# filixi/TCP-stack

Hardware: AMD Instinct MI355X
Metric: GiB/s device-resident TCP checksum over batched segments; % HBM roofline (higher is better)
Workload: dtype u16; 1 GPU; C2: 1M x 1460-B payload (1492-B images), fixed stride, device-resident; images_per_gpu=1048576, image_bytes=1492, bytes_per_gpu=1564475392, parallelism=shard1 (independent per-GPU batches, no collective)

## Files before the change

tcp-stack_amd/csrc/tcpck_device.h:

```cpp
#pragma once

#include <hip/hip_runtime.h>
#include <stdint.h>

#include "tcpck_internal.h"

namespace tcpck {
namespace dev {

using u32x4 = __attribute__((ext_vector_type(4))) unsigned int;

constexpr int kBlock = 256;
constexpr int kWavesPerBlock = kBlock / 64;

template <typename Kernel>
inline uint32_t resident_blocks_per_cu(Kernel kernel) {
  int nb = 0;
  if (hipOccupancyMaxActiveBlocksPerMultiprocessor(&nb, kernel, kBlock, 0) != hipSuccess || nb < 1) nb = 1;
  return static_cast<uint32_t>(nb);
}

inline uint32_t oversub_for(uint32_t requested, uint64_t bytes, uint64_t resident_waves, uint32_t max_m,
                            uint32_t min_run = 4u << 10) {
  if (requested) return requested;
// ... 78 lines not shown
  const uint32_t s = acc + w;
  return s + (s < w ? 1u : 0u);
}

template <int MODE>
__device__ __forceinline__ uint32_t accumulate(uint32_t acc, uint32_t w) {
  if constexpr (MODE == kRef) {
    return ref_add(acc, w);
  } else {
    return rfc_add(acc, w);
  }
}

template <int MODE>
__device__ __forceinline__ uint32_t fold_lane(uint32_t acc) {
  if constexpr (MODE == kRef) {
    return acc & 0xFFFFu;
  } else {
    acc = (acc & 0xFFFFu) + (acc >> 16);
    return (acc & 0xFFFFu) + (acc >> 16);
  }
}

template <int MODE>
__device__ __forceinline__ uint16_t finish(uint32_t sum) {
  if constexpr (MODE == kRef) {
    return static_cast<uint16_t>(~sum);
  } else {
    sum = (sum & 0xFFFFu) + (sum >> 16);
    sum = (sum & 0xFFFFu) + (sum >> 16);
    return static_cast<uint16_t>(~sum);
  }
}

template <int G>
__device__ __forceinline__ uint32_t group_sum(uint32_t x) {
#pragma unroll
  for (int m = G / 2; m >= 1; m >>= 1) x += __shfl_xor(x, m, 64);
  return x;
}

__device__ __forceinline__ uint32_t wave_inclusive_scan(uint32_t x) {
  x += __builtin_amdgcn_update_dpp(0, x, 0x111, 0xF, 0xF, false);
  x += __builtin_amdgcn_update_dpp(0, x, 0x112, 0xF, 0xF, false);
  x += __builtin_amdgcn_update_dpp(0, x, 0x114, 0xF, 0xF, false);
  x += __builtin_amdgcn_update_dpp(0, x, 0x118, 0xF, 0xF, false);
  x += __builtin_amdgcn_update_dpp(0, x, 0x142, 0xA, 0xF, false);
  x += __builtin_amdgcn_update_dpp(0, x, 0x143, 0xC, 0xF, false);
  return x;
}

__device__ __forceinline__ uint32_t read_lane(uint32_t x, uint32_t lane) {
  return static_cast<uint32_t>(__builtin_amdgcn_readlane(static_cast<int>(x), static_cast<int>(lane)));
}

__device__ __forceinline__ uint64_t read_lane64(uint64_t x, uint32_t lane) {
  const uint32_t lo = read_lane(static_cast<uint32_t>(x), lane);
  const uint32_t hi = read_lane(static_cast<uint32_t>(x >> 32), lane);
  return (static_cast<uint64_t>(hi) << 32) | lo;
}

template <bool EXACT = false>
__device__ __forceinline__ uint32_t words_before(uint32_t r, uint32_t x, uint32_t y, uint32_t z, uint32_t w) {
  const uint32_t nw = r >> 1;
  uint32_t h = 0;
  auto both = [](uint32_t d) -> uint32_t { return EXACT ? (d & 0xFFFFu) + (d >> 16) : d + (d >> 16); };
  if (nw >= 2) h += both(x);
  if (nw >= 4) h += both(y);
  if (nw >= 6) h += both(z);
  if (nw & 1) {
    const uint32_t d = nw == 1 ? x : (nw == 3 ? y : (nw == 5 ? z : w));
    h += d & 0xFFFFu;
  }
  return h;
}

template <int U, int MODE>
__device__ __forceinline__ uint32_t wave_image_sum(const uint8_t *arena, uint64_t start, uint32_t len,
                                                   bool exclude_field) {
  const uint32_t lane = threadIdx.x & 63;
  const uint64_t a0 = align16_rel(arena, start);
  const uint8_t *p0 = arena + a0;
  const int32_t lead = static_cast<int32_t>(start - a0);
  const int64_t span64 = lead + static_cast<int64_t>(len);
  const uint32_t nch = static_cast<uint32_t>((span64 + 15) >> 4);
  const int64_t field = exclude_field ? lead + 28 : -64;
  uint32_t acc = 0;
  for (uint32_t i0 = lane; i0 < nch; i0 += 64 * U) {
    u32x4 v[U];
#pragma unroll
    for (int u = 0; u < U; ++u) {
      const uint32_t i = i0 + u * 64;
      v[u] = load16_nt(p0 + 16 * static_cast<uint64_t>(i < nch ? i : nch - 1));
    }
#pragma unroll
    for (int u = 0; u < U; ++u) {
      const int64_t rel = 16 * static_cast<int64_t>(i0 + u * 64);
      const int32_t lo = static_cast<int32_t>(min(max(lead - rel, int64_t{0}), int64_t{16}));
      const int32_t hi = static_cast<int32_t>(min(max(span64 - rel, int64_t{0}), int64_t{16}));
      uint32_t wm = word_mask(lo, hi);
      const int64_t fb = field - rel;
      if (fb >= 0 && fb < 16) wm &= ~(1u << (fb >> 1));
      u32x4 w = v[u];
      if (wm != 0xFFu) w = apply_mask(w, wm);
      acc = accumulate<MODE>(acc, w.x);
      acc = accumulate<MODE>(acc, w.y);
// ... 27 lines not shown
                                         uint64_t t1, uint64_t &r0, uint64_t &r1) {
  const uint32_t lane = threadIdx.x & 63;
  uint64_t lo[2] = {0, 0}, hi[2] = {count, count};
  const uint64_t t[2] = {t0, t1};
  while (hi[0] - lo[0] > 64 || hi[1] - lo[1] > 64) {
    uint64_t step[2], idx[2], v[2];
#pragma unroll
    for (int i = 0; i < 2; ++i) {
      step[i] = hi[i] - lo[i] > 64 ? (hi[i] - lo[i] + 63) / 64 : 1;
      idx[i] = lo[i] + lane * step[i];
      v[i] = idx[i] < hi[i] ? offsets[idx[i]] : 0;
    }
#pragma unroll
    for (int i = 0; i < 2; ++i) {
      if (hi[i] - lo[i] <= 64) continue;
      const bool below = idx[i] < hi[i] && v[i] - base < t[i];
      const uint32_t c = __popcll(__ballot(below));
      const uint64_t nlo = c ? lo[i] + (c - 1) * step[i] + 1 : lo[i];
      hi[i] = min(hi[i], lo[i] + c * step[i]);
      lo[i] = nlo;
    }
  }
  uint64_t v[2];
#pragma unroll
  for (int i = 0; i < 2; ++i) {
    const uint64_t idx = lo[i] + lane;
    v[i] = idx < hi[i] ? offsets[idx] : 0;
  }
  const bool b0 = lo[0] + lane < hi[0] && v[0] - base < t0;
  const bool b1 = lo[1] + lane < hi[1] && v[1] - base < t1;
  r0 = lo[0] + __popcll(__ballot(b0));
  r1 = lo[1] + __popcll(__ballot(b1));
}

__device__ __forceinline__ void count_split(uint64_t wid, uint64_t q, uint64_t r, uint64_t &kb, uint64_t &ke) {
  kb = wid * q + (wid < r ? wid : r);
  ke = kb + q + (wid < r ? 1u : 0u);
}

__device__ __forceinline__ uint32_t xcd_block(uint32_t b, uint32_t nb) {
  const uint32_t q = nb >> 3, r = nb & 7u, x = b & 7u;
  return (x < r ? x * (q + 1) : r * (q + 1) + (x - r) * q) + (b >> 3);
}

__device__ __forceinline__ uint32_t xcd_chunk_block(uint32_t b, uint32_t nb, uint32_t lc) {
  const uint32_t full = (nb >> (3 + lc)) << (3 + lc);
  if (b >= full) return b;
  const uint32_t i = b >> 3;
  return ((((i >> lc) << 3) + (b & 7u)) << lc) + (i & ((1u << lc) - 1u));
}

constexpr uint32_t kOrderDefault = 0xFFu;
constexpr uint32_t kOrderXcd = 0xFEu;
__device__ __forceinline__ uint32_t ordered_block(uint32_t b, uint32_t nb, uint32_t lc) {
  if (lc == kOrderDefault) return b;
  if (lc == kOrderXcd) return xcd_block(b, nb);
  return xcd_chunk_block(b, nb, lc);
}


}
}
```

tcp-stack_amd/csrc/tcpck_internal.h:

```cpp
#pragma once

#include <hip/hip_runtime.h>
#include <stdint.h>

namespace tcpck {

enum Op : int { kChecksum = 0, kFill = 1, kVerify = 2 };
enum Mode : int { kRef = 0, kRfc1071 = 1 };

enum SegShape : int {
  kShapeSmall = 0,
  kShapeMss = 1,
  kShapeJumbo = 2,
  kShapeWave2 = 3,
  kShapeG32 = 4,
  kShapeG4 = 5,
  kShapeW4 = 6,
  kShapeW8 = 7,
  kShapeW16 = 8,
  kShapeW16U4 = 9,
  kShapeW2 = 10,
  kNumShapes = 11
};

struct SegArgs {
  uint8_t *arena;
  const uint64_t *offsets;
  const uint32_t *lengths;
  uint64_t stride;
  uint64_t base;
  uint64_t count;
  void *out;
  uint32_t len;
  uint32_t oversub;
  uint32_t order;
  uint32_t rot;
};

SegShape shape_for_len(uint64_t typical_len);
hipError_t launch_seg(int op, int mode, bool fixed, SegShape shape, const SegArgs &a,
                      uint32_t num_cus, hipStream_t stream);

struct RunArgs {
  uint8_t *arena;
  const uint64_t *offsets;
  const uint32_t *lengths;
  uint64_t stride;
  uint32_t len;
  uint64_t base;
  uint64_t count;
  void *out;
  uint32_t oversub;
  uint64_t total_bytes;
  uint32_t blocks_per_cu;
  int mode;
  uint8_t *hdr;
  uint64_t *dbg;
};

struct FixedStreamArgs {
  uint8_t *arena;
  uint64_t stride;
  uint64_t count;
  void *out;
  uint64_t *dbg;
  uint32_t blocks_per_cu;
  uint32_t oversub;
  uint64_t per_wave;
  uint64_t rem;
  uint32_t order;
  int mode;
  uint32_t defer_field;
  uint8_t *side;
  uint32_t side_nt;
};

struct GroupStreamArgs {
  uint8_t *arena;
  uint32_t len;
  uint64_t count;
  void *out;
  uint32_t oversub;
  uint32_t order;
  uint64_t per_wave;
  uint64_t rem;
};
bool gstream_applies(const uint8_t *arena, uint64_t stride, uint32_t len);
constexpr int kGstreamDefaultLoads = 0x80;
constexpr int kGstreamWriteBack = 0x401;
hipError_t launch_gstream(int op, int variant, const GroupStreamArgs &a, uint32_t num_cus, hipStream_t stream);

hipError_t launch_rstream(int op, int variant, const FixedStreamArgs &a, uint32_t num_cus, hipStream_t stream);
hipError_t launch_vvstream(int op, int variant, bool fixed, const RunArgs &a, uint32_t num_cus, hipStream_t stream);
hipError_t launch_rvstream(int op, int variant, const RunArgs &a, uint32_t num_cus, hipStream_t stream);
bool sstream_fixed_applies(uint64_t stride, uint32_t len);
hipError_t launch_sstream(int op, int variant, bool fixed, const RunArgs &a, uint32_t num_cus, hipStream_t stream);
struct SegmentArgs {
  const uint8_t *payload;
  uint8_t *images;
  uint64_t payload_bytes;
  uint64_t count;
  uint16_t *out;
  uint64_t per_wave, rem;
  uint32_t seg;
  uint32_t stride;
  uint32_t nchunk, magic, shift;
  uint32_t hdr[8];
  uint32_t seq0;
  uint32_t order;
};
hipError_t launch_segment(int mode, int variant, SegmentArgs a, uint32_t oversub, uint32_t num_cus,
                          hipStream_t stream);
struct AckArgs {
  uint8_t *arena;
  const uint64_t *offsets;
  uint64_t stride;
  uint64_t count;
  const uint32_t *acks;
  uint32_t ack;
  uint16_t *out;
};
hipError_t launch_set_ack(int mode, const AckArgs &a, uint32_t num_cus, hipStream_t stream);

// ... 35 lines not shown
```

tcp-stack_amd/csrc/tcpck_rstream.hip:

```cpp
#include "tcpck_device.h"

namespace tcpck {

namespace {

using dev::kBlock;
using dev::kWavesPerBlock;
using dev::u32x4;

template <int U, int OP, bool STAMP, int PRIO = 0, int FLAV = 0, int MODE = kRef>
__global__ void __launch_bounds__(kBlock) rstream_kernel(FixedStreamArgs a) {
  constexpr bool SECT = OP == kFill && (FLAV & 32) != 0;
  __shared__ u32x4 s_sec[kWavesPerBlock][SECT ? 32 * 4 : 1];
  const uint32_t lane = threadIdx.x & 63;
  const uint32_t wv = static_cast<uint32_t>(__builtin_amdgcn_readfirstlane(static_cast<int>(threadIdx.x >> 6)));
  const uint32_t bid = dev::ordered_block(blockIdx.x, gridDim.x, a.order);
  const uint64_t wid = static_cast<uint64_t>(bid) * kWavesPerBlock +
                       static_cast<uint32_t>(__builtin_amdgcn_readfirstlane(static_cast<int>(threadIdx.x >> 6)));
  uint64_t t_start = 0;
  if (STAMP) t_start = __builtin_amdgcn_s_memrealtime();
  if (PRIO) {
    uint32_t hw;
    asm volatile("s_getreg_b32 %0, hwreg(HW_REG_HW_ID)" : "=s"(hw));
    const uint32_t slot = hw & 0xFu;
    if (PRIO == 1) {
      if (slot >= 6) {
        __builtin_amdgcn_s_setprio(3);
      } else if (slot >= 4) {
        __builtin_amdgcn_s_setprio(2);
      } else if (slot >= 2) {
        __builtin_amdgcn_s_setprio(1);
      }
    } else if (slot >= 4) {
      __builtin_amdgcn_s_setprio(1);
    }
  }
  uint64_t kb, ke;
  dev::count_split(wid, a.per_wave, a.rem, kb, ke);
  if (kb >= ke) return;
  const uint32_t S = static_cast<uint32_t>(a.stride);
  const uint64_t s0 = kb * S;
  const uint64_t A0 = dev::align128_rel(a.arena, s0);
  const uint32_t lead = static_cast<uint32_t>(s0 - A0);
  const uint32_t span = lead + static_cast<uint32_t>(ke - kb) * S;
  const uint32_t nsteps = (span + 1023) >> 10;
  const uint32_t last_chunk = (span - 1) >> 4;
  const uint8_t *base = a.arena + A0;

  const auto rsrc = dev::make_rsrc(base, (last_chunk + 1) << 4);
  uint32_t nl = lead + 28;
  auto load_step = [&](uint32_t st) -> u32x4 {
    if constexpr ((FLAV & 128) != 0 && OP == kFill) {
      const uint32_t sb = st << 10;
      uint64_t m = 0;
      while (nl < sb + 1024 && nl < span) {
        m |= uint64_t{0xF} << (((nl & ~63u) - sb) >> 4);
        nl += S;
      }
      if ((m >> lane) & 1u) {
        typedef unsigned v4u __attribute__((ext_vector_type(4)));
        const v4u v = __builtin_amdgcn_raw_buffer_load_b128(rsrc, static_cast<int>(lane << 4), static_cast<int>(sb), 0);
        return u32x4{v.x, v.y, v.z, v.w};
      }
      return dev::load16_buf_nt(rsrc, lane << 4, sb);
    } else if constexpr (FLAV & 2) {
      if constexpr (FLAV & 8) {
        typedef unsigned v4u __attribute__((ext_vector_type(4)));
        const v4u v = __builtin_amdgcn_raw_buffer_load_b128(rsrc, static_cast<int>(lane << 4), static_cast<int>(st << 10), 0);
        return u32x4{v.x, v.y, v.z, v.w};
      } else {
        return dev::load16_buf_nt(rsrc, lane << 4, st << 10);
      }
    } else {
      const uint32_t ci = min((st << 6) + lane, last_chunk);
      return dev::load16_nt(base + 16 * static_cast<uint64_t>(ci));
    }
  };

  const uint32_t nimg = static_cast<uint32_t>(ke - kb);
  uint32_t nb = lead + S;
  uint32_t jn = 1;
  uint32_t nf = lead + 28;
  uint32_t jf = 0;
  uint32_t fstage = 0;
  uint32_t ns = lead + 28;
  uint32_t js = 0;
  const bool end_flush = SECT && (FLAV & 64) != 0 && nimg <= 32;
  uint32_t carry = 0;
  uint32_t p_last = 0;
  uint32_t stage = 0;
  uint32_t out_rel = 0;

  auto flush = [&](uint32_t n) {
    if (lane < n) {
      const uint64_t k = kb + out_rel + lane;
      const uint16_t c = static_cast<uint16_t>(stage);
      if constexpr (OP == kVerify) {
        static_cast<uint8_t *>(a.out)[k] = (c == 0) ? 1 : 0;
      } else {
        if (a.out) static_cast<uint16_t *>(a.out)[k] = c;
// ... 108 lines not shown
        }
      }
      const uint32_t tot = (FLAV & 1) ? dev::ref_chunk_sum_dot(w) : dev::ref_chunk_sum(w);
      const uint32_t incl = dev::wave_inclusive_scan(tot);
      while (nb < sb + 1024 && jn < nimg) {
        const uint32_t rel = nb - sb;
        const uint32_t lb = rel >> 4;
        const uint32_t r = rel & 15u;
        uint32_t P = carry + dev::read_lane(incl, lb) - dev::read_lane(tot, lb);
        if (r)
          P += dev::words_before<MODE == kRfc1071>(r, dev::read_lane(w.x, lb), dev::read_lane(w.y, lb), dev::read_lane(w.z, lb),
                            dev::read_lane(w.w, lb));
        emit(jn - 1, P - p_last);
        p_last = P;
        nb += S;
        ++jn;
      }
      carry += dev::read_lane(incl, 63);
      ring[u] = load_step(st + U);
    }
  }
  emit(nimg - 1, carry - p_last);
  if constexpr (SECT) {
    if (end_flush) {
      for (uint32_t j0 = 0; j0 < nimg; j0 += 16) flush_sect(j0, min(nimg - j0, 16u));
    } else if (nimg & 15u) {
      flush_sect(nimg & ~15u, nimg & 15u);
    }
  }
  const uint32_t pending = nimg - out_rel;
  if (pending) flush(pending);
  if (STAMP && lane == 0 && a.dbg) {
    uint32_t hw_id, xcc_id;
    asm volatile("s_getreg_b32 %0, hwreg(HW_REG_HW_ID)" : "=s"(hw_id));
    asm volatile("s_getreg_b32 %0, hwreg(HW_REG_XCC_ID)" : "=s"(xcc_id));
    a.dbg[4 * wid] = t_start;
    a.dbg[4 * wid + 1] = __builtin_amdgcn_s_memrealtime();
    a.dbg[4 * wid + 2] = hw_id;
    a.dbg[4 * wid + 3] = xcc_id;
  }
}

template <int U, int OP, bool STAMP, int PRIO = 0, int FLAV = 0, int MODE = kRef>
hipError_t launch_one(const FixedStreamArgs &a, uint32_t num_cus, hipStream_t stream) {
  static const uint32_t per_cu = dev::resident_blocks_per_cu(rstream_kernel<U, OP, STAMP, PRIO, FLAV, MODE>);
  const uint32_t cap = (a.blocks_per_cu && a.blocks_per_cu < per_cu) ? a.blocks_per_cu : per_cu;
  const uint64_t resident = static_cast<uint64_t>(cap) * num_cus;
  uint64_t blocks = resident * dev::oversub_for(a.oversub, a.count * a.stride, resident * kWavesPerBlock, 1024);
  const uint64_t need = (a.count + kWavesPerBlock - 1) / kWavesPerBlock;
  if (!a.oversub && a.stride >= 3584 && a.count < 2 * blocks * kWavesPerBlock) blocks = need;
  if (blocks > need) blocks = need;
  if (blocks == 0) return hipSuccess;
  FixedStreamArgs b = a;
  b.per_wave = a.count / (blocks * kWavesPerBlock);
  b.rem = a.count % (blocks * kWavesPerBlock);
  hipLaunchKernelGGL((rstream_kernel<U, OP, STAMP, PRIO, FLAV, MODE>), dim3(static_cast<uint32_t>(blocks)), dim3(kBlock), 0,
                     stream, b);
  return hipGetLastError();
}

template <int U, bool STAMP, int PRIO = 0, int FLAV = 0, int MODE = kRef>
hipError_t dispatch(int op, const FixedStreamArgs &a, uint32_t num_cus, hipStream_t s) {
  switch (op) {
    case kChecksum: return launch_one<U, kChecksum, STAMP, PRIO, FLAV, MODE>(a, num_cus, s);
    case kFill: return launch_one<U, kFill, STAMP, PRIO, FLAV, MODE>(a, num_cus, s);
    case kVerify: return launch_one<U, kVerify, STAMP, PRIO, FLAV, MODE>(a, num_cus, s);
    default: return hipErrorInvalidValue;
  }
}

}

hipError_t launch_rstream(int op, int variant, const FixedStreamArgs &a, uint32_t num_cus, hipStream_t stream) {
  if (a.stride < 16 || a.count == 0) return hipErrorInvalidValue;
  const uint64_t max_run = ((a.count + 2047) / 2048 + 1) * a.stride + 128;
  if (max_run >= (uint64_t{1} << 31)) return hipErrorInvalidValue;
  if (a.mode != kRef) {
    if (variant != 20 || a.stride >= (1u << 17)) return hipErrorInvalidValue;
    FixedStreamArgs b = a;
    b.order = 4u;
    return dispatch<4, false, 0, 263, kRfc1071>(op, b, num_cus, stream);
  }
  if (variant == 20) {
    FixedStreamArgs b = a;
    b.order = 4u;
    return dispatch<4, false, 0, 263>(op, b, num_cus, stream);
  }
#ifdef TCPCK_PROBE
  switch (variant) {
    case 0: return dispatch<4, false>(op, a, num_cus, stream);
    case 1: return dispatch<2, false>(op, a, num_cus, stream);
    case 2: return dispatch<8, false>(op, a, num_cus, stream);
    case 3: return op == kChecksum ? launch_one<4, kChecksum, true>(a, num_cus, stream) : hipErrorInvalidValue;
    case 4: return dispatch<4, false, 1>(op, a, num_cus, stream);
    case 5: return dispatch<4, false, 2>(op, a, num_cus, stream);
    case 6: return dispatch<8, false, 1>(op, a, num_cus, stream);
    case 7: return op == kChecksum ? launch_one<4, kChecksum, true, 1>(a, num_cus, stream) : hipErrorInvalidValue;
    case 8: return dispatch<2, false, 1>(op, a, num_cus, stream);
    case 9: return dispatch<4, false, 0, 1>(op, a, num_cus, stream);
    case 10: return dispatch<4, false, 0, 3>(op, a, num_cus, stream);
    case 11: return dispatch<4, false, 0, 2>(op, a, num_cus, stream);
    case 12: return dispatch<2, false, 0, 3>(op, a, num_cus, stream);
    case 13: return dispatch<8, false, 0, 3>(op, a, num_cus, stream);
    case 21: {
      FixedStreamArgs b = a;
      b.order = dev::kOrderXcd;
      return dispatch<4, false, 0, 7>(op, b, num_cus, stream);
    }
    case 22: {
      FixedStreamArgs b = a;
      b.order = 4u;
      return dispatch<4, false, 0, 11>(op, b, num_cus, stream);
    }
    case 27: {
      if (a.stride < 128 || a.defer_field) return hipErrorInvalidValue;
      FixedStreamArgs b = a;
      b.order = 4u;
      return dispatch<4, false, 0, 39>(op, b, num_cus, stream);
    }
    case 28: {
      if (a.stride < 128 || a.defer_field) return hipErrorInvalidValue;
      FixedStreamArgs b = a;
      b.order = 4u;
      return dispatch<4, false, 0, 103>(op, b, num_cus, stream);
    }
    case 33: case 34: {
      if (op != kFill || a.stride < 128 || a.defer_field || !a.side) return hipErrorInvalidValue;
      FixedStreamArgs b = a;
      b.order = 4u;
      return variant == 33 ? launch_one<4, kFill, false, 0, 807>(b, num_cus, stream)
                           : launch_one<4, kFill, false, 0, 871>(b, num_cus, stream);
    }
    case 29: case 30: {
      if (op != kFill || !a.defer_field || a.stride < 64) return hipErrorInvalidValue;
      FixedStreamArgs b = a;
      b.order = 4u;
      return variant == 29 ? launch_one<4, kFill, false, 0, 135>(b, num_cus, stream)
                           : launch_one<4, kFill, false, 0, 7>(b, num_cus, stream);
    }
// ... 30 lines not shown
```

tcp-stack_amd/csrc/tcpck_vvstream.hip:

```cpp
#include <type_traits>

#include "tcpck_device.h"
#include "tcpck_internal.h"

namespace tcpck {

namespace {

using dev::kBlock;
using dev::kWavesPerBlock;
using dev::u32x4;

constexpr uint32_t kRound = 256;
constexpr uint32_t kRing = 512;
constexpr uint32_t kMirror = 64;

struct VVArgs {
  uint8_t *arena;
  const uint64_t *offsets;
  const uint32_t *lengths;
  uint64_t base;
  uint64_t count;
  void *out;
  uint64_t per_wave, rem;
  uint32_t stride;
  uint32_t len;
  uint32_t order;
  uint32_t keep_first;
  uint32_t defer_field;
  uint64_t *dbg;
};

#ifdef TCPCK_PROBE
__device__ __forceinline__ uint64_t stamp_after(uint32_t dep) {
  uint64_t t;
  asm volatile("s_memrealtime %0\n\ts_waitcnt lgkmcnt(0)" : "=s"(t) : "v"(dep));
  return t;
}
#endif

__device__ __forceinline__ u32x4 zero_word(u32x4 w, uint32_t wi) {
  const uint32_t keep = (wi & 1u) ? 0x0000FFFFu : 0xFFFF0000u;
  const uint32_t di = wi >> 1;
  w.x &= di == 0 ? keep : 0xFFFFFFFFu;
  w.y &= di == 1 ? keep : 0xFFFFFFFFu;
  w.z &= di == 2 ? keep : 0xFFFFFFFFu;
  w.w &= di == 3 ? keep : 0xFFFFFFFFu;
  return w;
}

[[maybe_unused]] __device__ __forceinline__ u32x4 put_word(u32x4 w, uint32_t wi, uint32_t v) {
  const uint32_t sh = (wi & 1u) << 4;
  const uint32_t m = ~(0xFFFFu << sh), x = (v & 0xFFFFu) << sh;
  const uint32_t di = wi >> 1;
  w.x = di == 0 ? (w.x & m) | x : w.x;
  w.y = di == 1 ? (w.y & m) | x : w.y;
  w.z = di == 2 ? (w.z & m) | x : w.z;
  w.w = di == 3 ? (w.w & m) | x : w.w;
  return w;
}

[[maybe_unused]] __device__ __forceinline__ void store16_chunk_wt(__amdgpu_buffer_rsrc_t r, uint32_t voff, u32x4 v) {
  typedef unsigned v4u __attribute__((ext_vector_type(4)));
  __builtin_amdgcn_raw_buffer_store_b128(v4u{v.x, v.y, v.z, v.w}, r, static_cast<int>(voff), 0, 19);
}

template <int U, int OP, int SPLIT, int LAYOUT, bool KEEP = false, int MODE = kRef, bool BLK = false>
__global__ void __launch_bounds__(kBlock) vvstream_kernel(VVArgs a) {
  constexpr bool FIXED = LAYOUT != 0;
  constexpr bool GAP = LAYOUT == 2;
  static_assert(!BLK || (OP == kFill && !GAP && MODE == kRef && !KEEP), "BLK: reference-mode FILL, no gaps");
  constexpr uint32_t kMinFill = BLK ? 64u : 30u;
  __shared__ u32x4 s_blk[kWavesPerBlock][BLK ? 4 : 1];
  __shared__ uint32_t s_end[kWavesPerBlock][FIXED ? 1 : kRing + kMirror];
  __shared__ __attribute__((aligned(16))) uint32_t s_pre[kWavesPerBlock][MODE == kRef ? 256 : 512];
  __shared__ uint32_t s_fld[kWavesPerBlock][OP == kFill ? 64 : 1];
  const uint32_t lane = threadIdx.x & 63;
  const uint32_t wv = static_cast<uint32_t>(__builtin_amdgcn_readfirstlane(static_cast<int>(threadIdx.x >> 6)));
  const uint64_t W = static_cast<uint64_t>(gridDim.x) * kWavesPerBlock;
  const uint32_t bid = dev::ordered_block(blockIdx.x, gridDim.x, a.order);
  const uint64_t wid = static_cast<uint64_t>(bid) * kWavesPerBlock + wv;
  const uint64_t N = a.count;
#ifdef TCPCK_PROBE
  const uint64_t t_start = a.dbg ? __builtin_amdgcn_s_memrealtime() : 0;
  uint64_t t_desc = 0, t_first = 0;
#endif
  const uint32_t S = a.stride;
  const uint32_t L = FIXED ? a.len : 0u;
  uint64_t kb, ke;
  if (FIXED || SPLIT == 1) {
    dev::count_split(wid, a.per_wave, a.rem, kb, ke);
  } else {
    const uint64_t first = a.offsets[0] - a.base;
    const uint64_t total = a.offsets[N - 1] - a.base + a.lengths[N - 1] - first;
    const uint64_t q = total / W, rm = total % W;
    dev::find_two(a.offsets, a.base, N, first + q * wid + rm * wid / W,
                  first + q * (wid + 1) + rm * (wid + 1) / W, kb, ke);
    if (wid == 0) kb = 0;
    if (wid + 1 == W) ke = N;
  }
  if (kb >= ke) return;

  uint64_t s0, s1;
  if constexpr (FIXED) {
    s0 = kb * S;
    s1 = (ke - 1) * S + L;
  } else {
    s0 = a.offsets[kb] - a.base;
    s1 = a.offsets[ke - 1] - a.base + a.lengths[ke - 1];
  }
  uint8_t *const arena = a.arena;
  const uint64_t A0 = dev::align128_rel(arena, s0);
  const uint32_t nimg = static_cast<uint32_t>(ke - kb);
  const uint32_t nv = GAP ? 2 * nimg : nimg;
  bool bad = !(s1 >= s0 && s1 - A0 < (uint64_t{1} << 31));
#ifdef TCPCK_PROBE
  if (a.dbg) t_desc = stamp_after(static_cast<uint32_t>(s1 - A0));
#endif

  auto store = [&](uint64_t k, uint32_t sum, uint64_t start) {
    const uint16_t c = dev::finish<MODE>(sum);
    if constexpr (OP == kVerify) {
      static_cast<uint8_t *>(a.out)[k] = (c == 0) ? 1 : 0;
    } else {
      if (a.out) static_cast<uint16_t *>(a.out)[k] = c;
      if (OP == kFill) *reinterpret_cast<uint16_t *>(arena + start + 28) = c;
    }
  };
  auto store_rel = [&](uint64_t k, uint32_t sum, uint32_t start_rel, __amdgpu_buffer_rsrc_t r) {
    const uint16_t c = dev::finish<MODE>(sum);
    if constexpr (OP == kVerify) {
      static_cast<uint8_t *>(a.out)[k] = (c == 0) ? 1 : 0;
    } else {
      if (a.out) static_cast<uint16_t *>(a.out)[k] = c;
      if (OP == kFill && !a.defer_field) dev::store16_field(r, start_rel + 28, c);
    }
  };

  if (!bad) {
    const uint32_t lead = static_cast<uint32_t>(s0 - A0);
    const uint32_t span = static_cast<uint32_t>(s1 - A0);
    const uint32_t nsteps = (span + 1023) >> 10;
    const uint32_t last_chunk = span > 0 ? (span - 1) >> 4 : 0;
    int64_t blo = 0, bhi = 0;
    uint32_t extent = (last_chunk + 1) << 4;
    if constexpr (BLK) {
      const uint64_t b0 = FIXED ? 0 : a.offsets[0] - a.base;
      const uint64_t b1 = FIXED ? (N - 1) * S + L : a.offsets[N - 1] - a.base + a.lengths[N - 1];
      blo = static_cast<int64_t>(b0) - static_cast<int64_t>(A0);
      bhi = static_cast<int64_t>(b1) - static_cast<int64_t>(A0);
      const int64_t want = min(static_cast<int64_t>((span + 63u) & ~63u), bhi & ~int64_t{15});
      if (want > static_cast<int64_t>(extent)) extent = static_cast<uint32_t>(want);
    }
    const auto rsrc = dev::make_rsrc(arena + A0, extent);
    auto whole = [&](uint32_t b) { return static_cast<int64_t>(b) >= blo && static_cast<int64_t>(b) + 64 <= bhi; };
    uint32_t stage_f = 0;
    auto load_step = [&](uint32_t st) -> u32x4 {
      if constexpr (KEEP) {
        typedef unsigned v4u __attribute__((ext_vector_type(4)));
        const v4u v = __builtin_amdgcn_raw_buffer_load_b128(rsrc, static_cast<int>(lane << 4), static_cast<int>(st << 10), 0);
        return u32x4{v.x, v.y, v.z, v.w};
      } else {
        return dev::load16_buf_nt(rsrc, lane << 4, st << 10);
      }
    };
    uint32_t *ring_end = s_end[wv];
    u32x4 *pre4 = reinterpret_cast<u32x4 *>(s_pre[wv]);
    const uint16_t *pre16 = reinterpret_cast<const uint16_t *>(s_pre[wv]);
    uint32_t *fld = s_fld[wv];
    if constexpr (OP == kFill) {
      fld[lane] = 0;
      __builtin_amdgcn_wave_barrier();
    }

    uint32_t carry = 0, p_last = 0, jn = 0, fj = 0;
    uint32_t e_last = lead;
    u32x4 ring[U];
#pragma unroll
    for (int u = 0; u < U; ++u) {
      if (u == 0 && a.keep_first && (lane < 8 || a.keep_first == 2)) {
        typedef unsigned v4u __attribute__((ext_vector_type(4)));
        const v4u v = __builtin_amdgcn_raw_buffer_load_b128(rsrc, static_cast<int>(lane << 4), 0, 0);
        ring[0] = u32x4{v.x, v.y, v.z, v.w};
      } else {
        ring[u] = load_step(static_cast<uint32_t>(u));
      }
    }

    const uint32_t *lens = FIXED ? nullptr : a.lengths + kb;
    auto load_round = [&](uint32_t r, uint32_t (&d)[4]) {
#pragma unroll
      for (int i = 0; i < 4; ++i) {
        const uint32_t j = r * kRound + 4 * lane + i;
        d[i] = j < nimg ? lens[j] : 0u;
      }
    };
    uint32_t loaded = FIXED ? nv : 0;
    uint32_t pos = lead;
    bool short_fill = false;
    bool al4 = (lead & 3u) == 0 && (!FIXED || ((S & 3u) == 0 && (!GAP || (L & 3u) == 0)));
    auto fill_round = [&]() {
      const uint32_t r = loaded / kRound;
      uint32_t d[4];
      load_round(r, d);
      al4 = al4 && __ballot(((d[0] | d[1] | d[2] | d[3]) & 3u) != 0) == 0;
      if constexpr (MODE == kRfc1071) {
        bad = bad || __ballot((d[0] | d[1] | d[2] | d[3]) >= (1u << 17)) != 0;
      }
      const uint32_t e1 = d[0], e2 = e1 + d[1], e3 = e2 + d[2], e4 = e3 + d[3];
      const uint32_t incl = dev::wave_inclusive_scan(e4);
      const uint32_t ex = pos + incl - e4;
      if constexpr (OP == kFill) {
        const uint32_t jb = r * kRound + 4 * lane;
        bool sh = false;
#pragma unroll
        for (int i = 0; i < 4; ++i) sh |= (jb + i < nimg) && d[i] < kMinFill;
        short_fill |= __ballot(sh) != 0;
      }
      const uint32_t jb = r * kRound + 4 * lane;
      const uint32_t v0 = jb < nimg ? ex + e1 : ~0u, v1 = jb + 1 < nimg ? ex + e2 : ~0u;
      const uint32_t v2 = jb + 2 < nimg ? ex + e3 : ~0u, v3 = jb + 3 < nimg ? ex + e4 : ~0u;
      const uint32_t si = (r * kRound) % kRing + 4 * lane;
      ring_end[si] = v0;
      ring_end[si + 1] = v1;
      ring_end[si + 2] = v2;
      ring_end[si + 3] = v3;
      if (si < kMirror) {
        ring_end[kRing + si] = v0;
        ring_end[kRing + si + 1] = v1;
        ring_end[kRing + si + 2] = v2;
        ring_end[kRing + si + 3] = v3;
      }
      pos = pos + dev::read_lane(incl, 63);
      loaded += kRound;
      if (loaded >= nimg) {
        const uint32_t sn = loaded % kRing + lane;
        ring_end[sn] = ~0u;
        if (sn < kMirror) ring_end[kRing + sn] = ~0u;
      }
      __builtin_amdgcn_wave_barrier();
    };
    if constexpr (!FIXED) {
      fill_round();
      if constexpr (OP == kFill) {
        if (nimg > kRound) {
          uint32_t sum = 0;
          bool sh = false;
          for (uint32_t j = lane; j < nimg; j += 64) {
            const uint32_t l = lens[j];
            sum += l;
            sh |= l < kMinFill || (MODE == kRfc1071 && l >= (1u << 17));
          }
          short_fill = short_fill || __ballot(sh) != 0;
          bad = bad || short_fill || lead + dev::group_sum<64>(sum) != span;
        } else {
          bad = bad || short_fill || pos != span;
        }
      }
    } else {
      if constexpr (OP == kFill) bad = L < kMinFill;
    }
    auto end_of = [&](uint32_t j) -> uint32_t {
      if constexpr (GAP) {
        return lead + (j >> 1) * S + (j & 1u) * L;
      } else if constexpr (FIXED) {
        return lead + (j + 1) * S;
      } else {
        return ring_end[j % kRing];
      }
    };
    auto ends_at = [&](uint32_t jn0) -> uint32_t {
      if constexpr (FIXED) {
        const uint32_t j = jn0 + lane;
        return j < nv ? end_of(j) : ~0u;
      } else {
        return ring_end[jn0 % kRing + lane];
      }
    };

    auto stream_run = [&](auto al4_tag) {
      constexpr bool AL4 = decltype(al4_tag)::value;
      for (uint32_t g = 0; g < nsteps && !bad; g += U) {
  #pragma unroll
        for (int u = 0; u < U; ++u) {
          const uint32_t st = g + u;
          const uint32_t sb = st << 10;
          const uint32_t c = sb + (lane << 4);
          u32x4 w = ring[u];
          const u32x4 raw = w;
          if (sb == 0 || sb + 1024 > span) {
            const int32_t lo = min(max(static_cast<int32_t>(lead) - static_cast<int32_t>(c), 0), 16);
            const int32_t hi = min(max(static_cast<int32_t>(span) - static_cast<int32_t>(c), 0), 16);
            w = dev::apply_mask(w, dev::word_mask(lo, hi));
          }
          if (!FIXED && jn + 66 > loaded && loaded < nimg) fill_round();
          uint32_t j = jn + lane;
          uint32_t e = ends_at(jn);
          if constexpr (OP == kFill) {
            const uint32_t i = fj + lane;
            uint32_t f;
            if constexpr (FIXED)
              f = lead + i * S + 28;
            else
              f = (i == 0 ? lead : (i < nimg ? end_of(i - 1) : span)) + 28;
            const bool inf = i < nimg && f < sb + 1024;
            const uint64_t bf = __ballot(inf);
            if (bf) {
              if (inf) fld[(f - sb) >> 4] = ((f & 15u) >> 1) + 1u;
              __builtin_amdgcn_wave_barrier();
              const uint32_t q = fld[lane];
              if (q) {
                fld[lane] = 0u;
                w = zero_word(w, q - 1u);
              }
              __builtin_amdgcn_wave_barrier();
              fj += static_cast<uint32_t>(__popcll(bf));
            }
          }
          const uint32_t q1 = dev::dot2_u16(w.x, 0u);
          const uint32_t q2 = dev::dot2_u16(w.y, q1);
          const uint32_t q3 = dev::dot2_u16(w.z, q2);
          const uint32_t tot = dev::dot2_u16(w.w, q3);
#ifdef TCPCK_PROBE
          if (a.dbg && st == 0) t_first = stamp_after(tot);
#endif
          const uint32_t incl = dev::wave_inclusive_scan(tot);
          bool table = false;
          for (;;) {
            const bool inb = e < sb + 1024;
            const uint64_t bal = __ballot(inb);
            if (!bal) break;
            if (!table) {
              const uint32_t p0 = carry + incl - tot;
              const uint32_t b1 = p0 + q1, b2 = p0 + q2, b3 = p0 + q3;
              if constexpr (AL4) {
                pre4[lane] = u32x4{p0, b1, b2, b3};
              } else if constexpr (MODE == kRfc1071) {
                pre4[2 * lane] = u32x4{p0, p0 + (w.x & 0xFFFFu), b1, b1 + (w.y & 0xFFFFu)};
                pre4[2 * lane + 1] = u32x4{b2, b2 + (w.z & 0xFFFFu), b3, b3 + (w.w & 0xFFFFu)};
              } else
                pre4[lane] = u32x4{__builtin_amdgcn_perm(p0 + w.x, p0, 0x05040100u),
                                   __builtin_amdgcn_perm(b1 + w.y, b1, 0x05040100u),
                                   __builtin_amdgcn_perm(b2 + w.z, b2, 0x05040100u),
// ... 17 lines not shown
                  if (a.out) static_cast<uint16_t *>(a.out)[kb + j] = c;
                  const uint32_t f = start + 28;
                  if (f >= sb) {
                    fld[(f - sb) >> 4] = 0x80000000u | (((f & 15u) >> 1) << 16) | c;
                  } else if (whole(f & ~63u)) {
                    reinterpret_cast<uint16_t *>(s_blk[wv])[(f & 63u) >> 1] = c;
                  } else {
                    dev::store16_field(rsrc, f, c);
                  }
                }
              } else if (inb && (!GAP || (j & 1u))) {
                store_rel(kb + (GAP ? j >> 1 : j), P - pprev, start, rsrc);
              }
            } else {
              if (inb && (!GAP || (j & 1u))) store(kb + (GAP ? j >> 1 : j), P - pprev, 0);
            }
            p_last = dev::read_lane(P, cnt - 1);
            e_last = dev::read_lane(e, cnt - 1);
            jn += cnt;
            if (cnt < 64) break;
            if (!FIXED && jn + 66 > loaded && loaded < nimg) fill_round();
            j = jn + lane;
            e = ends_at(jn);
          }
          if constexpr (BLK) {
            __builtin_amdgcn_wave_barrier();
            if (stage_f != 0 && stage_f < e_last) {
              if (lane < 4 && whole(stage_f & ~63u)) store16_chunk_wt(rsrc, (stage_f & ~63u) + 16 * lane, s_blk[wv][lane]);
              stage_f = 0;
            }
            const uint32_t v = fld[lane];
            const uint64_t bv = __ballot(v != 0);
            if (bv) {
              const uint32_t cb = sb + ((lane & ~3u) << 4);
              if ((bv >> (lane & ~3u)) & 0xFull) {
                if (whole(cb))
                  store16_chunk_wt(rsrc, sb + (lane << 4), v ? put_word(raw, (v >> 16) & 7u, v) : raw);
                else if (v)
                  dev::store16_field(rsrc, sb + (lane << 4) + (((v >> 16) & 7u) << 1), static_cast<uint16_t>(v));
              }
              if (v) fld[lane] = 0u;
            }
            if (jn < nv) {
              const uint32_t f = e_last + 28;
              if (f >= sb && f < sb + 1024) {
                const uint32_t cb = f & ~63u;
                if (((sb + (lane << 4)) & ~63u) == cb) s_blk[wv][lane & 3u] = raw;
                stage_f = f;
              }
            }
          }
          __builtin_amdgcn_wave_barrier();
          carry += dev::read_lane(incl, 63);
          ring[u] = load_step(st + U);
        }
      }
    };
    if (al4 && (FIXED || loaded >= nimg))
      stream_run(std::true_type{});
    else
      stream_run(std::false_type{});
    if constexpr (!FIXED) bad = bad || pos != span || loaded < nimg;
    if (BLK && !bad && jn < nv) {
      const uint16_t c = dev::finish<MODE>(carry - p_last);
      if (lane == 0 && a.out) static_cast<uint16_t *>(a.out)[kb + jn] = c;
      const uint32_t f = e_last + 28;
      if (whole(f & ~63u)) {
        if (lane == 0) reinterpret_cast<uint16_t *>(s_blk[wv])[(f & 63u) >> 1] = c;
        __builtin_amdgcn_wave_barrier();
        if (lane < 4) store16_chunk_wt(rsrc, (f & ~63u) + 16 * lane, s_blk[wv][lane]);
      } else if (lane == 0) {
        dev::store16_field(rsrc, f, c);
      }
      jn = nv - 1 == jn ? nv : jn;
    }
    if (!bad && jn < nv) {
      const uint32_t rem = nv - jn;
      for (uint32_t i = lane; i < rem; i += 64) {
        const uint32_t v = jn + i;
        if (!GAP || (v & 1u)) store_rel(kb + (GAP ? v >> 1 : v), i == 0 ? carry - p_last : 0u, i == 0 ? e_last : span, rsrc);
      }
      jn = nv;
    }
    bad = bad || jn != nv;
  }
#ifdef TCPCK_PROBE
  if (a.dbg && lane == 0) {
    uint32_t hw_id, xcc_id;
    asm volatile("s_getreg_b32 %0, hwreg(HW_REG_HW_ID)" : "=s"(hw_id));
    asm volatile("s_getreg_b32 %0, hwreg(HW_REG_XCC_ID)" : "=s"(xcc_id));
    uint64_t *d = a.dbg + 8 * wid;
    d[0] = t_start;
    d[1] = t_desc;
    d[2] = t_first;
    d[3] = __builtin_amdgcn_s_memrealtime();
    d[4] = hw_id | (static_cast<uint64_t>(xcc_id) << 32);
    d[5] = ke - kb;
    d[6] = s1 - s0;
    d[7] = 0;
  }
#endif
  if (bad) {
    for (uint64_t k = kb; k < ke; ++k) {
      const uint64_t start = FIXED ? k * S : a.offsets[k] - a.base;
      const uint32_t len = FIXED ? L : a.lengths[k];
      if (OP == kFill && len < 30) continue;
      const uint32_t sum = dev::wave_image_sum<2, MODE>(arena, start, len, OP == kFill);
      if (lane == 0) store(k, sum, start);
    }
  }
}

template <int U, int OP, int SPLIT, int LAYOUT, bool KEEP = false, int MODE = kRef, bool BLK = false>
hipError_t launch_one(const RunArgs &s, uint32_t oversub, int flags, uint32_t num_cus, hipStream_t stream) {
  static const uint32_t per_cu = dev::resident_blocks_per_cu(vvstream_kernel<U, OP, SPLIT, LAYOUT, KEEP, MODE, BLK>);
  const uint64_t resident = static_cast<uint64_t>(per_cu) * num_cus;
  uint64_t blocks = resident * (oversub ? oversub : 1);
  const uint64_t need = (s.count + kWavesPerBlock - 1) / kWavesPerBlock;
  if (blocks > need) blocks = need;
  if (blocks == 0) return hipSuccess;
  VVArgs a{};
  a.arena = s.arena;
  a.offsets = s.offsets;
  a.lengths = s.lengths;
  a.base = s.base;
  a.count = s.count;
  a.out = s.out;
  a.per_wave = s.count / (blocks * kWavesPerBlock);
  a.rem = s.count % (blocks * kWavesPerBlock);
  a.stride = static_cast<uint32_t>(s.stride);
  a.len = s.len;
  a.order = (flags & 8) ? 4u : dev::kOrderDefault;
  a.keep_first = (flags & 16) ? ((flags & 256) ? 2u : 1u) : 0u;
  a.defer_field = (flags & 64) ? 1u : 0u;
  a.dbg = s.dbg;
  hipLaunchKernelGGL((vvstream_kernel<U, OP, SPLIT, LAYOUT, KEEP, MODE, BLK>), dim3(static_cast<uint32_t>(blocks)),
                     dim3(kBlock), 0, stream, a);
  return hipGetLastError();
}

template <int U, int SPLIT, int LAYOUT>
hipError_t dispatch(int op, const RunArgs &a, uint32_t oversub, int flags, uint32_t num_cus, hipStream_t s) {
  if (a.mode != kRef) {
    switch (op) {
      case kChecksum: return launch_one<U, kChecksum, SPLIT, LAYOUT, false, kRfc1071>(a, oversub, flags, num_cus, s);
      case kVerify: return launch_one<U, kVerify, SPLIT, LAYOUT, false, kRfc1071>(a, oversub, flags, num_cus, s);
      case kFill: return launch_one<U, kFill, SPLIT, LAYOUT, false, kRfc1071>(a, oversub, flags, num_cus, s);
      default: return hipErrorInvalidValue;
    }
  }
  switch (op) {
    case kChecksum: return launch_one<U, kChecksum, SPLIT, LAYOUT>(a, oversub, flags, num_cus, s);
    case kVerify: return launch_one<U, kVerify, SPLIT, LAYOUT>(a, oversub, flags, num_cus, s);
    case kFill:
#ifdef TCPCK_PROBE
      if constexpr (LAYOUT != 2)
        if (flags & 128) return launch_one<U, kFill, SPLIT, LAYOUT, false, kRef, true>(a, oversub, flags, num_cus, s);
#endif
      return (flags & 32) ? launch_one<U, kFill, SPLIT, LAYOUT, true>(a, oversub, flags, num_cus, s)
                          : launch_one<U, kFill, SPLIT, LAYOUT>(a, oversub, flags, num_cus, s);
    default: return hipErrorInvalidValue;
  }
}

}

hipError_t launch_vvstream(int op, int variant, bool fixed, const RunArgs &a, uint32_t num_cus,
                           hipStream_t stream) {
  if (a.count == 0) return hipSuccess;
  if (fixed && (a.len == 0 || a.stride < a.len || a.stride > (1u << 24))) return hipErrorInvalidValue;
  const bool gap = fixed && a.stride != a.len;
  const uint64_t bytes = fixed ? a.count * a.stride : a.total_bytes;
  uint32_t m = a.oversub ? a.oversub : 1;
  int flags = variant & 248;
  if ((flags & 64) && (op != kFill || !a.out)) return hipErrorInvalidValue;
#ifdef TCPCK_PROBE
  if ((flags & 128) && (op != kFill || a.mode != kRef || gap || (flags & 96))) return hipErrorInvalidValue;
#else
  if (flags & 128) return hipErrorInvalidValue;
#endif
  variant &= 7;
#ifdef TCPCK_PROBE
// ... 30 lines not shown
```

Before: 6950 GiB/s.

## Specialize block ordering, scalarize kernel args, and peel stream loop edges

Makes the rstream block-ordering policy a compile-time constant and passes the grid block count as a kernel argument instead of reading gridDim. Kernel argument structs are reordered and pinned to scalar registers, and the first offset and length loads are made wave-uniform and issued early. In vvstream, the ring-buffer streaming loop is split into a steady-state body with no edge masking plus peeled prologue and epilogue steps, so the first/last masking branch drops out of the hot loop. The aim is fewer scalar and vector instructions per step, at the cost of larger code and more complex tail handling.

```diff
diff --git a/tcp-stack_amd/csrc/tcpck_device.h b/tcp-stack_amd/csrc/tcpck_device.h
--- a/tcp-stack_amd/csrc/tcpck_device.h
+++ b/tcp-stack_amd/csrc/tcpck_device.h
@@ -154,6 +154,13 @@
 
 __device__ __forceinline__ uint32_t read_lane(uint32_t x, uint32_t lane) {
   return static_cast<uint32_t>(__builtin_amdgcn_readlane(static_cast<int>(x), static_cast<int>(lane)));
+}
+
+__device__ __forceinline__ uint32_t uniform32(uint32_t x) {
+  return static_cast<uint32_t>(__builtin_amdgcn_readfirstlane(static_cast<int>(x)));
+}
+__device__ __forceinline__ uint64_t uniform64(uint64_t x) {
+  return (static_cast<uint64_t>(uniform32(static_cast<uint32_t>(x >> 32))) << 32) | uniform32(static_cast<uint32_t>(x));
 }
 
 __device__ __forceinline__ uint64_t read_lane64(uint64_t x, uint32_t lane) {
@@ -287,7 +294,9 @@
 
 constexpr uint32_t kOrderDefault = 0xFFu;
 constexpr uint32_t kOrderXcd = 0xFEu;
+template <int ORDER = -1>
 __device__ __forceinline__ uint32_t ordered_block(uint32_t b, uint32_t nb, uint32_t lc) {
+  if constexpr (ORDER >= 0) lc = static_cast<uint32_t>(ORDER);
   if (lc == kOrderDefault) return b;
   if (lc == kOrderXcd) return xcd_block(b, nb);
   return xcd_chunk_block(b, nb, lc);
diff --git a/tcp-stack_amd/csrc/tcpck_internal.h b/tcp-stack_amd/csrc/tcpck_internal.h
--- a/tcp-stack_amd/csrc/tcpck_internal.h
+++ b/tcp-stack_amd/csrc/tcpck_internal.h
@@ -60,15 +60,16 @@
 
 struct FixedStreamArgs {
   uint8_t *arena;
-  uint64_t stride;
+  uint64_t rem;
+  uint32_t per_wave;
+  uint32_t stride;
+  uint32_t nblocks;
+  uint32_t order;
+  void *out;
   uint64_t count;
-  void *out;
   uint64_t *dbg;
   uint32_t blocks_per_cu;
   uint32_t oversub;
-  uint64_t per_wave;
-  uint64_t rem;
-  uint32_t order;
   int mode;
   uint32_t defer_field;
   uint8_t *side;
diff --git a/tcp-stack_amd/csrc/tcpck_rstream.hip b/tcp-stack_amd/csrc/tcpck_rstream.hip
--- a/tcp-stack_amd/csrc/tcpck_rstream.hip
+++ b/tcp-stack_amd/csrc/tcpck_rstream.hip
@@ -8,13 +8,18 @@
 using dev::kWavesPerBlock;
 using dev::u32x4;
 
+constexpr int kPolicyFlav = 263;
+constexpr int kPolicyOrder = 4;
+constexpr int order_of(int flav) { return flav == kPolicyFlav ? kPolicyOrder : -1; }
+
 template <int U, int OP, bool STAMP, int PRIO = 0, int FLAV = 0, int MODE = kRef>
 __global__ void __launch_bounds__(kBlock) rstream_kernel(FixedStreamArgs a) {
+  constexpr int ORDER = order_of(FLAV);
   constexpr bool SECT = OP == kFill && (FLAV & 32) != 0;
   __shared__ u32x4 s_sec[kWavesPerBlock][SECT ? 32 * 4 : 1];
   const uint32_t lane = threadIdx.x & 63;
   const uint32_t wv = static_cast<uint32_t>(__builtin_amdgcn_readfirstlane(static_cast<int>(threadIdx.x >> 6)));
-  const uint32_t bid = dev::ordered_block(blockIdx.x, gridDim.x, a.order);
+  const uint32_t bid = dev::ordered_block<ORDER>(blockIdx.x, a.nblocks, a.order);
   const uint64_t wid = static_cast<uint64_t>(bid) * kWavesPerBlock +
                        static_cast<uint32_t>(__builtin_amdgcn_readfirstlane(static_cast<int>(threadIdx.x >> 6)));
   uint64_t t_start = 0;
@@ -35,17 +40,19 @@
       __builtin_amdgcn_s_setprio(1);
     }
   }
+  uint8_t *const arena = a.arena;
+  asm volatile("" ::"s"(arena));
   uint64_t kb, ke;
   dev::count_split(wid, a.per_wave, a.rem, kb, ke);
   if (kb >= ke) return;
-  const uint32_t S = static_cast<uint32_t>(a.stride);
+  const uint32_t S = a.stride;
   const uint64_t s0 = kb * S;
-  const uint64_t A0 = dev::align128_rel(a.arena, s0);
+  const uint64_t A0 = dev::align128_rel(arena, s0);
   const uint32_t lead = static_cast<uint32_t>(s0 - A0);
   const uint32_t span = lead + static_cast<uint32_t>(ke - kb) * S;
   const uint32_t nsteps = (span + 1023) >> 10;
   const uint32_t last_chunk = (span - 1) >> 4;
-  const uint8_t *base = a.arena + A0;
+  const uint8_t *base = arena + A0;
 
   const auto rsrc = dev::make_rsrc(base, (last_chunk + 1) << 4);
   uint32_t nl = lead + 28;
@@ -260,8 +267,12 @@
   if (blocks > need) blocks = need;
   if (blocks == 0) return hipSuccess;
   FixedStreamArgs b = a;
-  b.per_wave = a.count / (blocks * kWavesPerBlock);
+  const uint64_t per_wave = a.count / (blocks * kWavesPerBlock);
+  if (per_wave >> 32) return hipErrorInvalidValue;
+  b.per_wave = static_cast<uint32_t>(per_wave);
   b.rem = a.count % (blocks * kWavesPerBlock);
+  b.nblocks = static_cast<uint32_t>(blocks);
+  if (order_of(FLAV) >= 0) b.order = static_cast<uint32_t>(order_of(FLAV));
   hipLaunchKernelGGL((rstream_kernel<U, OP, STAMP, PRIO, FLAV, MODE>), dim3(static_cast<uint32_t>(blocks)), dim3(kBlock), 0,
                      stream, b);
   return hipGetLastError();
@@ -285,14 +296,10 @@
   if (max_run >= (uint64_t{1} << 31)) return hipErrorInvalidValue;
   if (a.mode != kRef) {
     if (variant != 20 || a.stride >= (1u << 17)) return hipErrorInvalidValue;
-    FixedStreamArgs b = a;
-    b.order = 4u;
-    return dispatch<4, false, 0, 263, kRfc1071>(op, b, num_cus, stream);
+    return dispatch<4, false, 0, kPolicyFlav, kRfc1071>(op, a, num_cus, stream);
   }
   if (variant == 20) {
-    FixedStreamArgs b = a;
-    b.order = 4u;
-    return dispatch<4, false, 0, 263>(op, b, num_cus, stream);
+    return dispatch<4, false, 0, kPolicyFlav>(op, a, num_cus, stream);
   }
 #ifdef TCPCK_PROBE
   switch (variant) {
diff --git a/tcp-stack_amd/csrc/tcpck_vvstream.hip b/tcp-stack_amd/csrc/tcpck_vvstream.hip
--- a/tcp-stack_amd/csrc/tcpck_vvstream.hip
+++ b/tcp-stack_amd/csrc/tcpck_vvstream.hip
@@ -20,14 +20,15 @@
   const uint64_t *offsets;
   const uint32_t *lengths;
   uint64_t base;
+  uint64_t per_wave, rem;
+  uint32_t nblocks;
+  uint32_t order;
+  uint32_t keep_first;
+  uint32_t stride;
+  uint32_t len;
+  uint32_t defer_field;
   uint64_t count;
   void *out;
-  uint64_t per_wave, rem;
-  uint32_t stride;
-  uint32_t len;
-  uint32_t order;
-  uint32_t keep_first;
-  uint32_t defer_field;
   uint64_t *dbg;
 };
 
@@ -77,8 +78,14 @@
   __shared__ uint32_t s_fld[kWavesPerBlock][OP == kFill ? 64 : 1];
   const uint32_t lane = threadIdx.x & 63;
   const uint32_t wv = static_cast<uint32_t>(__builtin_amdgcn_readfirstlane(static_cast<int>(threadIdx.x >> 6)));
-  const uint64_t W = static_cast<uint64_t>(gridDim.x) * kWavesPerBlock;
-  const uint32_t bid = dev::ordered_block(blockIdx.x, gridDim.x, a.order);
+  if constexpr (LAYOUT == 0)
+    asm volatile("" ::"s"(a.arena), "s"(a.offsets), "s"(a.lengths), "s"(a.base), "s"(a.per_wave), "s"(a.rem), "s"(a.nblocks),
+                 "s"(a.order), "s"(a.keep_first));
+  else
+    asm volatile("" ::"s"(a.arena), "s"(a.per_wave), "s"(a.rem), "s"(a.nblocks), "s"(a.order), "s"(a.keep_first),
+                 "s"(a.stride), "s"(a.len));
+  const uint64_t W = static_cast<uint64_t>(a.nblocks) * kWavesPerBlock;
+  const uint32_t bid = dev::ordered_block(blockIdx.x, a.nblocks, a.order);
   const uint64_t wid = static_cast<uint64_t>(bid) * kWavesPerBlock + wv;
   const uint64_t N = a.count;
 #ifdef TCPCK_PROBE
@@ -100,18 +107,33 @@
     if (wid + 1 == W) ke = N;
   }
   if (kb >= ke) return;
-
+  const uint32_t nimg = static_cast<uint32_t>(ke - kb);
+
+  const uint32_t *lens = FIXED ? nullptr : a.lengths + kb;
+  auto load_round = [&](uint32_t r, uint32_t (&d)[4]) {
+#pragma unroll
+    for (int i = 0; i < 4; ++i) {
+      const uint32_t j = r * kRound + 4 * lane + i;
+      d[i] = j < nimg ? lens[j] : 0u;
+    }
+  };
   uint64_t s0, s1;
+  uint32_t d_first[4] = {0u, 0u, 0u, 0u};
   if constexpr (FIXED) {
     s0 = kb * S;
     s1 = (ke - 1) * S + L;
   } else {
-    s0 = a.offsets[kb] - a.base;
-    s1 = a.offsets[ke - 1] - a.base + a.lengths[ke - 1];
+    uint64_t o0 = a.offsets[kb], o1 = a.offsets[ke - 1];
+    uint32_t l1 = a.lengths[ke - 1];
+    load_round(0u, d_first);
+    o0 = dev::uniform64(o0);
+    o1 = dev::uniform64(o1);
+    l1 = dev::uniform32(l1);
+    s0 = o0 - a.base;
+    s1 = o1 - a.base + l1;
   }
   uint8_t *const arena = a.arena;
   const uint64_t A0 = dev::align128_rel(arena, s0);
-  const uint32_t nimg = static_cast<uint32_t>(ke - kb);
   const uint32_t nv = GAP ? 2 * nimg : nimg;
   bool bad = !(s1 >= s0 && s1 - A0 < (uint64_t{1} << 31));
 #ifdef TCPCK_PROBE
@@ -175,34 +197,12 @@
 
     uint32_t carry = 0, p_last = 0, jn = 0, fj = 0;
     uint32_t e_last = lead;
-    u32x4 ring[U];
-#pragma unroll
-    for (int u = 0; u < U; ++u) {
-      if (u == 0 && a.keep_first && (lane < 8 || a.keep_first == 2)) {
-        typedef unsigned v4u __attribute__((ext_vector_type(4)));
-        const v4u v = __builtin_amdgcn_raw_buffer_load_b128(rsrc, static_cast<int>(lane << 4), 0, 0);
-        ring[0] = u32x4{v.x, v.y, v.z, v.w};
-      } else {
-        ring[u] = load_step(static_cast<uint32_t>(u));
-      }
-    }
-
-    const uint32_t *lens = FIXED ? nullptr : a.lengths + kb;
-    auto load_round = [&](uint32_t r, uint32_t (&d)[4]) {
-#pragma unroll
-      for (int i = 0; i < 4; ++i) {
-        const uint32_t j = r * kRound + 4 * lane + i;
-        d[i] = j < nimg ? lens[j] : 0u;
-      }
-    };
     uint32_t loaded = FIXED ? nv : 0;
     uint32_t pos = lead;
     bool short_fill = false;
     bool al4 = (lead & 3u) == 0 && (!FIXED || ((S & 3u) == 0 && (!GAP || (L & 3u) == 0)));
-    auto fill_round = [&]() {
+    auto write_round = [&](const uint32_t (&d)[4]) {
       const uint32_t r = loaded / kRound;
-      uint32_t d[4];
-      load_round(r, d);
       al4 = al4 && __ballot(((d[0] | d[1] | d[2] | d[3]) & 3u) != 0) == 0;
       if constexpr (MODE == kRfc1071) {
         bad = bad || __ballot((d[0] | d[1] | d[2] | d[3]) >= (1u << 17)) != 0;
@@ -240,8 +240,13 @@
       }
       __builtin_amdgcn_wave_barrier();
     };
+    auto fill_round = [&]() {
+      uint32_t d[4];
+      load_round(loaded / kRound, d);
+      write_round(d);
+    };
     if constexpr (!FIXED) {
-      fill_round();
+      write_round(d_first);
       if constexpr (OP == kFill) {
         if (nimg > kRound) {
           uint32_t sum = 0;
@@ -280,15 +285,22 @@
 
     auto stream_run = [&](auto al4_tag) {
       constexpr bool AL4 = decltype(al4_tag)::value;
-      for (uint32_t g = 0; g < nsteps && !bad; g += U) {
+      u32x4 ring[U];
   #pragma unroll
-        for (int u = 0; u < U; ++u) {
-          const uint32_t st = g + u;
+      for (int u = 0; u < U; ++u) {
+        if (u == 0 && a.keep_first && (lane < 8 || a.keep_first == 2)) {
+          typedef unsigned v4u __attribute__((ext_vector_type(4)));
+          const v4u v = __builtin_amdgcn_raw_buffer_load_b128(rsrc, static_cast<int>(lane << 4), 0, 0);
+          ring[0] = u32x4{v.x, v.y, v.z, v.w};
+        } else {
+          ring[u] = load_step(static_cast<uint32_t>(u));
+        }
+      }
+      auto step = [&](u32x4 w, uint32_t st, const bool first, const bool last) {
           const uint32_t sb = st << 10;
           const uint32_t c = sb + (lane << 4);
-          u32x4 w = ring[u];
           const u32x4 raw = w;
-          if (sb == 0 || sb + 1024 > span) {
+          if ((first && sb == 0) || (last && sb + 1024 > span)) {
             const int32_t lo = min(max(static_cast<int32_t>(lead) - static_cast<int32_t>(c), 0), 16);
             const int32_t hi = min(max(static_cast<int32_t>(span) - static_cast<int32_t>(c), 0), 16);
             w = dev::apply_mask(w, dev::word_mask(lo, hi));
@@ -412,8 +424,33 @@
           }
           __builtin_amdgcn_wave_barrier();
           carry += dev::read_lane(incl, 63);
-          ring[u] = load_step(st + U);
+      };
+      uint32_t g = 0, slot = 0;
+      if (nsteps >= static_cast<uint32_t>(U)) {
+        for (; g + 2 * U <= nsteps && !bad; g += U) {
+  #pragma unroll
+          for (int u = 0; u < U; ++u) {
+            step(ring[u], g + u, u == 0, false);
+            ring[u] = load_step(g + u + U);
+          }
         }
+        slot = U - 1;
+  #pragma unroll
+        for (int u = 0; u < U - 1; ++u) {
+          if (bad || g + u + U >= nsteps) {
+            slot = static_cast<uint32_t>(u);
+            break;
+          }
+          step(ring[u], g + u, u == 0, false);
+          ring[u] = load_step(g + u + U);
+        }
+      }
+  #pragma unroll
+      for (int t = 0; t < 2 * U - 1; ++t) {
+        if (t < U && static_cast<uint32_t>(t) < slot) continue;
+        const uint32_t st = g + static_cast<uint32_t>(t);
+        if (bad || st >= nsteps) break;
+        step(ring[t % U], st, t == 0, true);
       }
     };
     if (al4 && (FIXED || loaded >= nimg))
@@ -488,6 +525,7 @@
   a.out = s.out;
   a.per_wave = s.count / (blocks * kWavesPerBlock);
   a.rem = s.count % (blocks * kWavesPerBlock);
+  a.nblocks = static_cast<uint32_t>(blocks);
   a.stride = static_cast<uint32_t>(s.stride);
   a.len = s.len;
   a.order = (flags & 8) ? 4u : dev::kOrderDefault;
```

Result: no change. 6966 GiB/s (median of 5 runs) (+0.2%).
